# serviceberry3/weiner_slamit_v2

Hardware: AMD Instinct MI355X
Metric: frames/sec ORB extract+match @640x480x8lvl (higher is better)
Workload: dtype u8; 1 GPU; BASELINE configs[1]: 640x480 8-level ORB extract (1000 features, FAST 20/7) + brute-force 256-bit Hamming best/second match vs the stream's previous frame; 256 independent streams per GPU per step; distinct_frame_pairs_per_gpu=16, parallelism=streams sharded over 1 GPU(s), no data-path collective

## Files before the change

### weiner_slamit_v2_amd/csrc/orb_kernels.hip

```cpp
#include <hip/hip_runtime.h>
#include <stdint.h>

#include <algorithm>

#include "orb_types.h"
#include "slamit_math.h"
#include "wave_ops.h"
#include "../../include/slamit.h"
#include "../../include/slamit_orb_pattern.h"

#define WAVE 64

__global__ __launch_bounds__(256) void resize_level_kernel(
    const uint8_t* __restrict__ src, int sw, int sh, size_t sstride, size_t sframe,
    uint8_t* __restrict__ dst, int dw, int dh, size_t dstride, size_t dframe,
    const int* __restrict__ xofs, const short* __restrict__ ialpha,
    const int* __restrict__ yofs, const short* __restrict__ ibeta) {
    const int x4 = (blockIdx.x * 64 + (threadIdx.x & 63)) * 4;
    const int y = blockIdx.y * 4 + (threadIdx.x >> 6);
    const int f = blockIdx.z;
    if (x4 >= dw || y >= dh) return;
    const uint8_t* S = src + (size_t)f * sframe;
    int sy = yofs[y];
    int sy0 = min(max(sy, 0), sh - 1), sy1 = min(max(sy + 1, 0), sh - 1);
// ... 1119 lines not shown
    }
#endif
}

template <int OCT_NT>
__global__ __launch_bounds__(OCT_NT) void octree_kernel(
    const OrbLevel* __restrict__ levels, int nlevels,
    const unsigned long long* __restrict__ cand, size_t cand_frame_stride,
    int* __restrict__ cand_count,
    uint32_t* __restrict__ ws_xy, uint16_t* __restrict__ ws_node,
    OrbLevelKp* __restrict__ lkp, size_t kp_frame_stride, int* __restrict__ kp_count,
    int node_cap, int key_cap, int level_override ) {
    extern __shared__ __attribute__((aligned(16))) unsigned char smem[];
    __shared__ int wave_tmp[OCT_NT / 64];
    __shared__ int s_vars[4];
    uint32_t* k_xy = reinterpret_cast<uint32_t*>(smem + orbk_octree_node_bytes(node_cap));
    uint16_t* k_nd = reinterpret_cast<uint16_t*>(k_xy + key_cap);
    const int level = level_override >= 0 ? level_override : blockIdx.y;
    const int frame = blockIdx.x;
    const OrbLevel& L = levels[level];
    const int kidx = frame * nlevels + level;
    const int n_raw = cand_count[kidx * ORB_CC_PAD];
    const int n_keys = min(n_raw, L.cand_cap);
    __syncthreads();
    if (threadIdx.x == 0) { cand_count[kidx * ORB_CC_PAD] = 0; cand_count[kidx * ORB_CC_PAD + 1] = n_raw; }
    const unsigned long long* K = cand + L.cand_off + (size_t)frame * cand_frame_stride;
    OrbLevelKp* OUT = lkp + L.kp_off + (size_t)frame * kp_frame_stride;
    if (n_keys == 0) {
        if (threadIdx.x == 0) kp_count[kidx] = 0;
        return;
    }
    if (n_keys <= key_cap)
        octree_body<OCT_NT, true>(L, K, n_keys, k_xy, k_nd, OUT, &kp_count[kidx], smem, node_cap, wave_tmp, s_vars);
    else
        octree_body<OCT_NT, false>(L, K, n_keys, ws_xy + L.cand_off + (size_t)frame * cand_frame_stride,
                                        ws_node + L.cand_off + (size_t)frame * cand_frame_stride, OUT, &kp_count[kidx], smem,
                                        node_cap, wave_tmp, s_vars);
}

struct DiscTable { signed char uv[64][32]; int n; };
__constant__ DiscTable c_disc;

static DiscTable make_disc() {
    static const int umax[16] = {15, 15, 15, 15, 14, 14, 14, 13, 13, 12, 11, 10, 9, 8, 6, 3};
    DiscTable t;
    for (int l = 0; l < 64; ++l) for (int k = 0; k < 32; ++k) t.uv[l][k] = 0;
    t.n = 0;
    for (int v = -15; v <= 15; ++v)
        for (int u = -umax[v < 0 ? -v : v]; u <= umax[v < 0 ? -v : v]; ++u) {
            t.uv[t.n & 63][2 * (t.n >> 6)] = (signed char)u; t.uv[t.n & 63][2 * (t.n >> 6) + 1] = (signed char)v;
            ++t.n;
        }
    return t;
}

#define IC_KP_PER_WAVE 8
#define IC_R 15
#define IC_ROWS (2 * IC_R + 1)
#define IC_PITCH 32

__global__ __launch_bounds__(256) void ic_angle_kernel(
    const OrbLevel* __restrict__ levels, int nlevels,
    const uint8_t* __restrict__ img0, size_t img0_stride, size_t img0_frame,
    const uint8_t* __restrict__ pyr,
    OrbLevelKp* __restrict__ lkp, size_t kp_frame_stride, const int* __restrict__ kp_count, int xcd_frames, int kblocks) {
    const int lane = threadIdx.x & 63;
    int level, frame, kb;
    if (xcd_frames) {
        const unsigned w = blockIdx.x, k = w >> 3, P = (unsigned)(nlevels * kblocks), fq = k / P, local = k - fq * P;
        frame = (int)(8u * fq + ((w + fq) & 7u));
        if (frame >= xcd_frames) return;
        level = (int)(local / (unsigned)kblocks); kb = (int)(local - (unsigned)level * (unsigned)kblocks);
    } else { level = blockIdx.y; frame = blockIdx.z; kb = blockIdx.x; }
    const OrbLevel& L = levels[level];
    const int count = kp_count[frame * nlevels + level];
    const int i0 = (kb * 4 + (threadIdx.x >> 6)) * IC_KP_PER_WAVE;
    if (i0 >= count) return;
    const uint8_t* src;
    int stride;
    if (level == 0) { src = img0 + (size_t)frame * img0_frame; stride = (int)img0_stride; }
    else { src = pyr + L.plane_off + (size_t)frame * L.plane_bytes; stride = L.stride; }
    __shared__ __attribute__((aligned(16))) uint8_t s_win[4][IC_KP_PER_WAVE][IC_ROWS * IC_PITCH];
    const int wvi = threadIdx.x >> 6;
    OrbLevelKp* kp0 = lkp + L.kp_off + (size_t)frame * kp_frame_stride;
    typedef unsigned ic_u4 __attribute__((ext_vector_type(4), aligned(1)));
    {
        const int lr = min(lane >> 1, IC_ROWS - 1), lc = lane & 1;
        const unsigned loff = __umul24((unsigned)lr, (unsigned)stride) + 16u * (unsigned)lc;
        ic_u4 ld[IC_KP_PER_WAVE];
#pragma unroll
        for (int k = 0; k < IC_KP_PER_WAVE; ++k) {
            const int i = min(i0 + k, count - 1);
            const uint8_t* corner = src + (__umul24((unsigned)(kp0[i].y - IC_R), (unsigned)stride) + (unsigned)(kp0[i].x - IC_R));
            ld[k] = *reinterpret_cast<const ic_u4*>(corner + loff);
        }
#pragma unroll
        for (int k = 0; k < IC_KP_PER_WAVE; ++k)
            if (lane < 2 * IC_ROWS) *reinterpret_cast<uint4*>(&s_win[wvi][k][lr * IC_PITCH + 16 * lc]) = make_uint4(ld[k].x, ld[k].y, ld[k].z, ld[k].w);
    }
    int off[12], wu[12], wv[12];
    {
        const uint4 t0 = *reinterpret_cast<const uint4*>(&c_disc.uv[lane][0]);
        const uint2 t1 = *reinterpret_cast<const uint2*>(&c_disc.uv[lane][16]);
        const uint32_t tw[6] = {t0.x, t0.y, t0.z, t0.w, t1.x, t1.y};
#pragma unroll
        for (int j = 0; j < 12; ++j) {
            const uint32_t pr = tw[j >> 1] >> (16 * (j & 1));
            const int u = (int)(signed char)(pr & 0xFFu), v = (int)(signed char)((pr >> 8) & 0xFFu);
            off[j] = (v + IC_R) * IC_PITCH + (u + IC_R); wu[j] = u; wv[j] = v;
        }
    }
    const float factorPI = (float)(3.14159265358979323846 / 180.f);
    wave_sync_lds();
    int val[IC_KP_PER_WAVE][12];
#pragma unroll
    for (int k = 0; k < IC_KP_PER_WAVE; ++k)
#pragma unroll
        for (int j = 0; j < 12; ++j) val[k][j] = s_win[wvi][k][off[j]];
    int V[2 * IC_KP_PER_WAVE];
#pragma unroll
    for (int k = 0; k < IC_KP_PER_WAVE; ++k) {
        int m10 = 0, m01 = 0;
#pragma unroll
        for (int j = 0; j < 12; ++j) { m10 += __mul24(wu[j], val[k][j]); m01 += __mul24(wv[j], val[k][j]); }
        V[2 * k] = m10; V[2 * k + 1] = m01;
    }
    {
        const bool b0 = lane & 1, b1 = lane & 2, b2 = lane & 4, b3 = lane & 8;
#pragma unroll
        for (int p = 0; p < 8; ++p) { const int a = V[2 * p], b = V[2 * p + 1]; V[p] = (b0 ? b : a) + dpp<0xB1>(b0 ? a : b); }
#pragma unroll
        for (int p = 0; p < 4; ++p) { const int a = V[2 * p], b = V[2 * p + 1]; V[p] = (b1 ? b : a) + dpp<0x4E>(b1 ? a : b); }
#pragma unroll
        for (int p = 0; p < 2; ++p) { const int a = V[2 * p], b = V[2 * p + 1]; V[p] = (b2 ? b : a) + dpp<0x1B>(dpp<0x141>(b2 ? a : b)); }
        { const int a = V[0], b = V[1]; V[0] = (b3 ? b : a) + dpp<0x141>(dpp<0x140>(b3 ? a : b)); }
    }
    __shared__ int s_rows[4][64];
    int* sr = s_rows[threadIdx.x >> 6];
    sr[lane] = V[0];
    wave_sync_lds();
    const int tot = (sr[lane & 15] + sr[(lane & 15) + 16]) + (sr[(lane & 15) + 32] + sr[(lane & 15) + 48]);
    const int my10 = tot, my01 = dpp<0xB1>(tot);
    if (lane < 2 * IC_KP_PER_WAVE && !(lane & 1) && i0 + (lane >> 1) < count) {
        const float ang = slamit_fast_atan2((float)my01, (float)my10);
        float sn, cs;
        slamit_sincosf(ang * factorPI, &sn, &cs);
        OrbLevelKp* kp = kp0 + i0 + (lane >> 1);
        kp->angle = ang; kp->cs = cs; kp->sn = sn;
    }
}

__device__ __forceinline__ int reflect101(int p, int len) {
    p = p < 0 ? -p : p;
    p = p >= len ? 2 * len - 2 - p : p;
    return min(max(p, 0), len - 1);
}


typedef unsigned short blur_us2 __attribute__((ext_vector_type(2)));
__device__ __forceinline__ uint32_t udot2(uint32_t a, uint32_t b, uint32_t c) {
    return __builtin_amdgcn_udot2(__builtin_bit_cast(blur_us2, a), __builtin_bit_cast(blur_us2, b), c, false);
}

__device__ __forceinline__ uint32_t blur_fetch(const uint8_t* S, unsigned sstride, bool whole, int w, int h, int gx0, int row) {
    const unsigned ro = (unsigned)reflect101(row, h) * sstride;
    if (whole) return *reinterpret_cast<const uint32_t*>(S + (ro + (unsigned)gx0));
    if (gx0 >= w + 3) return 0u;
    uint32_t v = 0;
#pragma unroll
    for (int j = 0; j < 4; ++j) v |= (uint32_t)S[ro + (unsigned)reflect101(gx0 + j, w)] << (8 * j);
    return v;
}

struct BlurCol { unsigned a0, a1, sel; };
__device__ __forceinline__ BlurCol blur_col(int g, int w, unsigned ss) {
#define BLUR_SEL(i0, i1, i2, i3) ((unsigned)(i0) | ((unsigned)(i1) << 8) | ((unsigned)(i2) << 16) | ((unsigned)(i3) << 24))
    BlurCol c;
    if (g < 0) { c.a0 = 0u; c.a1 = 4u; c.sel = BLUR_SEL(4, 3, 2, 1); }
    else if (g + 4 <= w) { c.a0 = c.a1 = (unsigned)g; c.sel = BLUR_SEL(0, 1, 2, 3); }
    else if (g < w) {
        const int q = w - g;
        unsigned idx[4];
#pragma unroll
        for (int j = 0; j < 4; ++j) idx[j] = (unsigned)(j < q ? 4 + j : 2 * q + 2 - j);
        c.a0 = (unsigned)(g - 4); c.a1 = (unsigned)g; c.sel = BLUR_SEL(idx[0], idx[1], idx[2], idx[3]);
    } else if (g <= w + 2) {
        const int t = g - w, gb = (w - 4) & ~3;
        unsigned idx[4];
#pragma unroll
        for (int j = 0; j < 4; ++j) idx[j] = j <= 2 - t ? (unsigned)(w - 2 - t - j - gb) : 0x0Cu;
        c.a0 = (unsigned)gb; c.a1 = min((unsigned)gb + 4u, ss - 4u); c.sel = BLUR_SEL(idx[0], idx[1], idx[2], idx[3]);
    } else { c.a0 = c.a1 = 0u; c.sel = BLUR_SEL(0x0C, 0x0C, 0x0C, 0x0C); }
#undef BLUR_SEL
    return c;
}
__device__ __forceinline__ uint32_t blur_fetch2(const uint8_t* S, unsigned ss, int h, int row, const BlurCol c) {
    const unsigned ro = __umul24((unsigned)reflect101(row, h), ss);
    return __builtin_amdgcn_perm(*reinterpret_cast<const uint32_t*>(S + (ro + c.a1)), *reinterpret_cast<const uint32_t*>(S + (ro + c.a0)), c.sel);
}

template <bool INTERIOR>
__device__ __forceinline__ void blur_strip(uint8_t (*in)[72], uint32_t (*rp)[64], const uint8_t* S, const size_t sstride, const bool aligned,
                                           uint8_t* D, const unsigned dstride, const int w, const int h, const int bx, const int by0, const int tid) {
    const int i0 = tid, i1 = tid + 256;
    const bool has1 = i1 < 22 * 18;
    const int r0 = i0 / 18, r1 = i1 / 18;
    const int g0 = bx - 4 + 4 * (i0 - r0 * 18), g1 = bx - 4 + 4 * (i1 - r1 * 18);
    const bool whole0 = aligned && g0 >= 0 && g0 + 4 <= w, whole1 = aligned && g1 >= 0 && g1 + 4 <= w;
    uint32_t* const st0 = reinterpret_cast<uint32_t*>(&in[r0][4 * (i0 - r0 * 18)]);
    uint32_t* const st1 = reinterpret_cast<uint32_t*>(&in[has1 ? r1 : 0][has1 ? 4 * (i1 - r1 * 18) : 0]);
    const unsigned ss = (unsigned)sstride;
    const BlurCol bc0 = blur_col(g0, w, ss), bc1 = blur_col(g1, w, ss);
    uint32_t v0 = INTERIOR ? *reinterpret_cast<const uint32_t*>(S + (__umul24((unsigned)(by0 + r0 - 3), ss) + (unsigned)g0))
                           : aligned ? blur_fetch2(S, ss, h, by0 + r0 - 3, bc0) : blur_fetch(S, ss, whole0, w, h, g0, by0 + r0 - 3);
    uint32_t v1 = !has1 ? 0u : INTERIOR ? *reinterpret_cast<const uint32_t*>(S + (__umul24((unsigned)(by0 + r1 - 3), ss) + (unsigned)g1))
                                        : aligned ? blur_fetch2(S, ss, h, by0 + r1 - 3, bc1) : blur_fetch(S, ss, whole1, w, h, g1, by0 + r1 - 3);
    *st0 = v0;
    if (has1) *st1 = v1;
    __syncthreads();
    const uint32_t TA = 18u | (34u << 8) | (49u << 16) | (55u << 24), TB = 49u | (34u << 8) | (18u << 16);
    const int cy = tid >> 4, cx4 = (tid & 15) * 4;
    const bool odd = cy & 1;
    const uint32_t k0 = odd ? (18u << 16) : (18u | (34u << 16)), k1 = odd ? (34u | (49u << 16)) : (49u | (55u << 16));
    const uint32_t k2 = odd ? (55u | (49u << 16)) : (49u | (34u << 16)), k3 = odd ? (34u | (18u << 16)) : 18u;
#pragma unroll 1
    for (int s = 0; s < BLUR_STEPS; ++s) {
        const int by = by0 + 16 * s;
        const bool more = s + 1 < BLUR_STEPS && (INTERIOR || by + 16 < h);
        if (more) {
            if (INTERIOR) {
                v0 = *reinterpret_cast<const uint32_t*>(S + (__umul24((unsigned)(by + 16 + r0 - 3), ss) + (unsigned)g0));
                if (has1) v1 = *reinterpret_cast<const uint32_t*>(S + (__umul24((unsigned)(by + 16 + r1 - 3), ss) + (unsigned)g1));
            } else {
                if (aligned) {
                    v0 = blur_fetch2(S, ss, h, by + 16 + r0 - 3, bc0);
                    if (has1) v1 = blur_fetch2(S, ss, h, by + 16 + r1 - 3, bc1);
                } else {
                    v0 = blur_fetch(S, ss, whole0, w, h, g0, by + 16 + r0 - 3);
                    if (has1) v1 = blur_fetch(S, ss, whole1, w, h, g1, by + 16 + r1 - 3);
                }
            }
        }
        if (tid < 11 * 16) {
            const int p = tid >> 4, c = (tid & 15) * 4;
            uint32_t o[2][4];
#pragma unroll
            for (int rr = 0; rr < 2; ++rr) {
                const uint32_t* pw = reinterpret_cast<const uint32_t*>(&in[2 * p + rr][c]);
                const uint32_t w0 = pw[0], w1 = pw[1], w2 = pw[2];
                o[rr][0] = __builtin_amdgcn_udot4(__builtin_amdgcn_alignbyte(w2, w1, 1), TB, __builtin_amdgcn_udot4(__builtin_amdgcn_alignbyte(w1, w0, 1), TA, 0u, false), false);
                o[rr][1] = __builtin_amdgcn_udot4(__builtin_amdgcn_alignbyte(w2, w1, 2), TB, __builtin_amdgcn_udot4(__builtin_amdgcn_alignbyte(w1, w0, 2), TA, 0u, false), false);
                o[rr][2] = __builtin_amdgcn_udot4(__builtin_amdgcn_alignbyte(w2, w1, 3), TB, __builtin_amdgcn_udot4(__builtin_amdgcn_alignbyte(w1, w0, 3), TA, 0u, false), false);
                o[rr][3] = __builtin_amdgcn_udot4(w2, TB, __builtin_amdgcn_udot4(w1, TA, 0u, false), false);
            }
            *reinterpret_cast<uint4*>(&rp[p][c]) = make_uint4(o[0][0] | (o[1][0] << 16), o[0][1] | (o[1][1] << 16),
                                                               o[0][2] | (o[1][2] << 16), o[0][3] | (o[1][3] << 16));
        }
        __syncthreads();
        if (more) {
            *st0 = v0;
            if (has1) *st1 = v1;
        }
        if (INTERIOR || (bx + cx4 < w && by + cy < h)) {
            const int pb = cy >> 1;
            const uint4 a0 = *reinterpret_cast<const uint4*>(&rp[pb][cx4]), a1 = *reinterpret_cast<const uint4*>(&rp[pb + 1][cx4]);
            const uint4 a2 = *reinterpret_cast<const uint4*>(&rp[pb + 2][cx4]), a3 = *reinterpret_cast<const uint4*>(&rp[pb + 3][cx4]);
#define BLUR_COL(f) min((udot2(a3.f, k3, udot2(a2.f, k2, udot2(a1.f, k1, udot2(a0.f, k0, 1u << 15)))) >> 16), 255u)
            const uint32_t out = BLUR_COL(x) | (BLUR_COL(y) << 8) | (BLUR_COL(z) << 16) | (BLUR_COL(w) << 24);
#undef BLUR_COL
            *reinterpret_cast<uint32_t*>(D + (__umul24((unsigned)(by + cy), dstride) + (unsigned)(bx + cx4))) = out;
        }
        if (!more) break;
        __syncthreads();
    }
}

__global__ __launch_bounds__(256) void blur_all_kernel(
    const OrbLevel* __restrict__ levels, const uint4* __restrict__ tiles,
    const uint8_t* __restrict__ img0, size_t img0_stride, size_t img0_frame,
    const uint8_t* __restrict__ pyr, uint8_t* __restrict__ blur, unsigned ntiles, unsigned inv_tiles, unsigned total) {
    __shared__ __attribute__((aligned(16))) uint8_t in[22][72];
    __shared__ __attribute__((aligned(16))) uint32_t rp[11][64];
    const int tid = threadIdx.x;
    const unsigned lin = blockIdx.x, per_xcd = (total + 7u) >> 3;
    const unsigned logical = (lin & 7u) * per_xcd + (lin >> 3);
    if (logical >= total) return;
    int frame = (int)__umulhi(logical, inv_tiles);
    if ((unsigned)frame * ntiles > logical) --frame;
    const uint4 tt = tiles[logical - (unsigned)frame * ntiles];
    const int level = (int)tt.x, bx = (int)tt.y, by0 = (int)tt.z;
    const OrbLevel& L = levels[level];
    const int w = L.w, h = L.h;
    const uint8_t* S;
    size_t sstride;
    if (level == 0) { S = img0 + (size_t)frame * img0_frame; sstride = img0_stride; }
    else { S = pyr + L.plane_off + (size_t)frame * L.plane_bytes; sstride = (size_t)L.stride; }
    const bool aligned = ((((uintptr_t)S) | sstride) & 3) == 0;
    uint8_t* D = blur + L.blur_off + (size_t)frame * L.blur_bytes;
    const bool interior = aligned && bx >= 4 && bx + 68 <= w && by0 >= 3 && by0 + ORB_BLUR_STRIP_H + 3 <= h;
    if (interior) blur_strip<true>(in, rp, S, sstride, aligned, D, (unsigned)L.stride, w, h, bx, by0, tid);
    else blur_strip<false>(in, rp, S, sstride, aligned, D, (unsigned)L.stride, w, h, bx, by0, tid);
}

template <bool EDGE>
__global__ __launch_bounds__(256) void blur_stream_kernel(
    const OrbLevel* __restrict__ levels, const uint4* __restrict__ tiles,
    const uint8_t* __restrict__ img0, size_t img0_stride, size_t img0_frame,
    const uint8_t* __restrict__ pyr, uint8_t* __restrict__ blur, unsigned ntiles) {
    const unsigned tile = blockIdx.x * 16u + (threadIdx.x >> 4);
    if (tile >= ntiles) return;
    const int frame = blockIdx.y;
    const uint4 tt = tiles[tile];
    const int level = (int)tt.x, by0 = (int)tt.z;
    const int x0 = (int)tt.y + 4 * (int)(threadIdx.x & 15);
    const OrbLevel& L = levels[level];
    const int h = L.h;
    const uint8_t* S;
    unsigned ss;
    if (level == 0) { S = img0 + (size_t)frame * img0_frame; ss = (unsigned)img0_stride; }
    else { S = pyr + L.plane_off + (size_t)frame * L.plane_bytes; ss = (unsigned)L.stride; }
    if (EDGE && x0 >= L.w) return;
    BlurCol bc[3];
    if (EDGE) {
#pragma unroll
        for (int k = 0; k < 3; ++k) bc[k] = blur_col(x0 - 4 + 4 * k, L.w, ss);
    } else S += x0 - 4;
    uint8_t* D = blur + L.blur_off + (size_t)frame * L.blur_bytes + x0;
    const unsigned ds = (unsigned)L.stride;
    const uint32_t TA = 18u | (34u << 8) | (49u << 16) | (55u << 24), TB = 49u | (34u << 8) | (18u << 16);
    const uint32_t kA0 = 18u | (34u << 16), kA1 = 49u | (55u << 16), kA2 = 49u | (34u << 16), kA3 = 18u;
    const uint32_t kB0 = 18u << 16, kB1 = 34u | (49u << 16), kB2 = 55u | (49u << 16), kB3 = 34u | (18u << 16);
    const int ylast = min(by0 + ORB_BLUR_STRIP_H, h) - 1;
    const int p0 = (by0 - 3) >> 1, p1 = (ylast + 3) >> 1;
    typedef unsigned blur_u3 __attribute__((ext_vector_type(3)));
    auto fetch = [&](int yy) -> blur_u3 {
        int r = yy < 0 ? -yy : yy;
        r = r >= h ? 2 * h - 2 - r : r;
        r = min(max(r, 0), h - 1);
        if (EDGE) {
            const uint8_t* R = S + __umul24((unsigned)r, ss);
            blur_u3 v;
            v.x = __builtin_amdgcn_perm(*reinterpret_cast<const uint32_t*>(R + bc[0].a1), *reinterpret_cast<const uint32_t*>(R + bc[0].a0), bc[0].sel);
            v.y = __builtin_amdgcn_perm(*reinterpret_cast<const uint32_t*>(R + bc[1].a1), *reinterpret_cast<const uint32_t*>(R + bc[1].a0), bc[1].sel);
            v.z = __builtin_amdgcn_perm(*reinterpret_cast<const uint32_t*>(R + bc[2].a1), *reinterpret_cast<const uint32_t*>(R + bc[2].a0), bc[2].sel);
            return v;
        }
        return *reinterpret_cast<const blur_u3*>(S + __umul24((unsigned)r, ss));
    };
    auto rowpass = [&](const blur_u3 v, uint32_t* o) {
        o[0] = __builtin_amdgcn_udot4(__builtin_amdgcn_alignbyte(v.z, v.y, 1), TB, __builtin_amdgcn_udot4(__builtin_amdgcn_alignbyte(v.y, v.x, 1), TA, 0u, false), false);
        o[1] = __builtin_amdgcn_udot4(__builtin_amdgcn_alignbyte(v.z, v.y, 2), TB, __builtin_amdgcn_udot4(__builtin_amdgcn_alignbyte(v.y, v.x, 2), TA, 0u, false), false);
        o[2] = __builtin_amdgcn_udot4(__builtin_amdgcn_alignbyte(v.z, v.y, 3), TB, __builtin_amdgcn_udot4(__builtin_amdgcn_alignbyte(v.y, v.x, 3), TA, 0u, false), false);
        o[3] = __builtin_amdgcn_udot4(v.z, TB, __builtin_amdgcn_udot4(v.y, TA, 0u, false), false);
    };
    uint32_t P0[4] = {0, 0, 0, 0}, P1[4] = {0, 0, 0, 0}, P2[4] = {0, 0, 0, 0}, P3[4];
    blur_u3 va = fetch(2 * p0), vb = fetch(2 * p0 + 1), va1 = fetch(2 * p0 + 2), vb1 = fetch(2 * p0 + 3), va2 = fetch(2 * p0 + 4), vb2 = fetch(2 * p0 + 5);
#pragma unroll 4
    for (int p = p0; p <= p1; ++p) {
        const blur_u3 ca = va, cb = vb;
        va = va1; vb = vb1; va1 = va2; vb1 = vb2;
        va2 = fetch(2 * p + 6); vb2 = fetch(2 * p + 7);
        uint32_t oa[4], ob[4];
        rowpass(ca, oa); rowpass(cb, ob);
#pragma unroll
        for (int j = 0; j < 4; ++j) P3[j] = oa[j] | (ob[j] << 16);
        const int ya = 2 * p - 3, yb = 2 * p - 2;
#define BLUR_OUT(k0, k1, k2, k3, j) min((udot2(P3[j], k3, udot2(P2[j], k2, udot2(P1[j], k1, udot2(P0[j], k0, 1u << 15)))) >> 16), 255u)
        if (ya >= by0 && ya <= ylast)
            *reinterpret_cast<uint32_t*>(D + __umul24((unsigned)ya, ds)) = BLUR_OUT(kA0, kA1, kA2, kA3, 0) | (BLUR_OUT(kA0, kA1, kA2, kA3, 1) << 8) | (BLUR_OUT(kA0, kA1, kA2, kA3, 2) << 16) | (BLUR_OUT(kA0, kA1, kA2, kA3, 3) << 24);
        if (yb >= by0 && yb <= ylast)
            *reinterpret_cast<uint32_t*>(D + __umul24((unsigned)yb, ds)) = BLUR_OUT(kB0, kB1, kB2, kB3, 0) | (BLUR_OUT(kB0, kB1, kB2, kB3, 1) << 8) | (BLUR_OUT(kB0, kB1, kB2, kB3, 2) << 16) | (BLUR_OUT(kB0, kB1, kB2, kB3, 3) << 24);
#undef BLUR_OUT
#pragma unroll
        for (int j = 0; j < 4; ++j) { P0[j] = P1[j]; P1[j] = P2[j]; P2[j] = P3[j]; }
    }
}

__constant__ __attribute__((aligned(16))) signed char c_pattern[SLAMIT_ORB_PATTERN_INTS];
#define DESC_KP_PER_WAVE 4
#define DESC_R 18
#define DESC_ROWS (2 * DESC_R + 1)
#define DESC_PITCH 48
#define DESC_LOADS 2

__global__ __launch_bounds__(256) void describe_kernel(
    const OrbLevel* __restrict__ levels, int nlevels,
    const uint8_t* __restrict__ blur,
    const OrbLevelKp* __restrict__ lkp, size_t kp_frame_stride, const int* __restrict__ kp_count,
    slamit_kp* __restrict__ out_kps, uint8_t* __restrict__ out_desc, int out_cap,
    int* __restrict__ out_n, int xcd_frames , int kblocks) {
    const int lane = threadIdx.x & 63;
    int level, frame, kb;
    if (xcd_frames) {
        const unsigned w = blockIdx.x, k = w >> 3, P = (unsigned)(nlevels * kblocks), fq = k / P, local = k - fq * P;
        frame = (int)(8u * fq + ((w + fq) & 7u));
        if (frame >= xcd_frames) return;
        level = (int)(local / (unsigned)kblocks); kb = (int)(local - (unsigned)level * (unsigned)kblocks);
    } else { level = blockIdx.y; frame = blockIdx.z; kb = blockIdx.x; }
    const int i0 = (kb * 4 + (threadIdx.x >> 6)) * DESC_KP_PER_WAVE;
    const OrbLevel& L = levels[level];
    const int* counts = kp_count + frame * nlevels;
    int offset = 0, total = 0;
    for (int l = 0; l < nlevels; ++l) {
        int c = counts[l];
        if (l < level) offset += c;
        total += c;
    }
    if (level == 0 && i0 == 0 && lane == 0) out_n[frame] = min(total, out_cap);
    const int count = counts[level];
    if (i0 >= count) return;
    const int4 pw = reinterpret_cast<const int4*>(c_pattern)[lane];
    const int pt[4] = {pw.x, pw.y, pw.z, pw.w};
    float px0[4], py0[4], px1[4], py1[4];
#pragma unroll
    for (int t = 0; t < 4; ++t) {
        px0[t] = (float)(signed char)(pt[t] & 0xFF); py0[t] = (float)(signed char)((pt[t] >> 8) & 0xFF);
        px1[t] = (float)(signed char)((pt[t] >> 16) & 0xFF); py1[t] = (float)(signed char)((pt[t] >> 24) & 0xFF);
    }
    const uint8_t* img = blur + L.blur_off + (size_t)frame * L.blur_bytes;
    const unsigned step = (unsigned)L.stride;
    const OrbLevelKp* KP = lkp + L.kp_off + (size_t)frame * kp_frame_stride;
    OrbLevelKp kp[DESC_KP_PER_WAVE];
#pragma unroll
    for (int k = 0; k < DESC_KP_PER_WAVE; ++k) kp[k] = KP[min(i0 + k, count - 1)];
    __shared__ __attribute__((aligned(16))) uint8_t s_patch[4][DESC_KP_PER_WAVE][DESC_ROWS * DESC_PITCH];
    const int wv = threadIdx.x >> 6;
    int lrow[DESC_LOADS], lcol[DESC_LOADS];
    unsigned poff[DESC_LOADS];
#pragma unroll
    for (int it = 0; it < DESC_LOADS; ++it) {
        const int idx = lane + 64 * it;
        lrow[it] = (int)(((unsigned)idx * 21846u) >> 16);
        lcol[it] = idx - 3 * lrow[it];
        poff[it] = __umul24((unsigned)min(lrow[it], DESC_ROWS - 1), step) + 16u * (unsigned)lcol[it];
    }
    const __amdgpu_buffer_rsrc_t rsrc = __builtin_amdgcn_make_buffer_rsrc(const_cast<uint8_t*>(img), 0, (unsigned)L.stride * (unsigned)L.h, 0x00020000);
    typedef unsigned desc_u4 __attribute__((ext_vector_type(4)));
    desc_u4 ld[DESC_KP_PER_WAVE][DESC_LOADS];
#pragma unroll
    for (int k = 0; k < DESC_KP_PER_WAVE; ++k) {
        const unsigned base = __umul24((unsigned)(kp[k].y - DESC_R), step) + (unsigned)((kp[k].x - DESC_R) & ~3);
#pragma unroll
        for (int it = 0; it < DESC_LOADS; ++it) ld[k][it] = __builtin_amdgcn_raw_buffer_load_b128(rsrc, (int)(base + poff[it]), 0, 0);
    }
#pragma unroll
    for (int k = 0; k < DESC_KP_PER_WAVE; ++k)
#pragma unroll
        for (int it = 0; it < DESC_LOADS; ++it)
            if (lrow[it] < DESC_ROWS) *reinterpret_cast<desc_u4*>(&s_patch[wv][k][__mul24(lrow[it], DESC_PITCH) + 16 * lcol[it]]) = ld[k][it];
    __builtin_amdgcn_fence(__ATOMIC_ACQ_REL, "wavefront");
    __builtin_amdgcn_wave_barrier();
    typedef float desc_f2 __attribute__((ext_vector_type(2)));
    const desc_f2 magic = {12582912.0f, 12582912.0f};
    const unsigned DESC_BIAS = 0x400000u * (unsigned)DESC_PITCH + 0x4B400000u;
    int tv0[DESC_KP_PER_WAVE][4], tv1[DESC_KP_PER_WAVE][4];
#pragma unroll
    for (int k = 0; k < DESC_KP_PER_WAVE; ++k) {
        const float a = kp[k].cs, b = kp[k].sn;
        const desc_f2 ba = {b, a}, anb = {a, -b};
        const uint8_t* center = &s_patch[wv][k][DESC_R * DESC_PITCH + DESC_R + ((kp[k].x - DESC_R) & 3)];
        const uint8_t* biased = center - DESC_BIAS;
#pragma unroll
        for (int t = 0; t < 4; ++t) {
            const desc_f2 p0 = {px0[t], px0[t]}, q0 = {py0[t], py0[t]}, p1 = {px1[t], px1[t]}, q1 = {py1[t], py1[t]};
            const desc_f2 m0 = (p0 * ba + q0 * anb) + magic, m1 = (p1 * ba + q1 * anb) + magic;
            tv0[k][t] = biased[__umul24(__float_as_uint(m0.x), (unsigned)DESC_PITCH) + __float_as_uint(m0.y)];
            tv1[k][t] = biased[__umul24(__float_as_uint(m1.x), (unsigned)DESC_PITCH) + __float_as_uint(m1.y)];
        }
    }
#pragma unroll
    for (int k = 0; k < DESC_KP_PER_WAVE; ++k) {
        const int i = i0 + k, o = offset + i;
        unsigned nib = 0;
#pragma unroll
        for (int t = 0; t < 4; ++t) nib |= (unsigned)(tv0[k][t] < tv1[k][t]) << t;
        unsigned other = __shfl_xor(nib, 1, WAVE);
        if (i >= count || o >= out_cap) continue;
        if ((lane & 1) == 0)
            out_desc[((size_t)frame * out_cap + o) * SLAMIT_DESC_BYTES + (lane >> 1)] = (uint8_t)(nib | (other << 4));
        if (lane == 0) {
            slamit_kp kk;
            float fx = (float)kp[k].x, fy = (float)kp[k].y;
            if (level != 0) { fx *= L.scale; fy *= L.scale; }
            kk.x = fx; kk.y = fy; kk.size = L.patch_size; kk.angle = kp[k].angle; kk.response = kp[k].response;
            kk.octave = level; kk.class_id = -1;
            out_kps[(size_t)frame * out_cap + o] = kk;
        }
    }
}

__global__ __launch_bounds__(256) void pad_level_kernel(const uint8_t* __restrict__ src, int w, int h,
                                                        size_t sstride, uint8_t* __restrict__ dst) {
    const int B = SLAMIT_EDGE_THRESHOLD;
    const int pw = w + 2 * B, ph = h + 2 * B;
    int x = blockIdx.x * 64 + (threadIdx.x & 63), y = blockIdx.y * 4 + (threadIdx.x >> 6);
    if (x >= pw || y >= ph) return;
    dst[(size_t)y * pw + x] = src[(size_t)reflect101(y - B, h) * sstride + reflect101(x - B, w)];
}

__global__ void decode_candidates_kernel(const OrbLevel* __restrict__ levels, int level,
                                         const unsigned long long* __restrict__ K, int n,
                                         unsigned long long* __restrict__ order_out, int* __restrict__ xys) {
    int k = blockIdx.x * blockDim.x + threadIdx.x;
    if (k >= n) return;
    const OrbLevel& L = levels[level];
    unsigned long long c = K[k];
    unsigned order = (unsigned)c;
    int lx = order & 63, ly = (order >> 6) & 63, cell = order >> 12;
    int ci = cell / L.nCols, cj = cell - ci * L.nCols;
    xys[3 * k + 0] = cj * L.wCell + lx;
    xys[3 * k + 1] = ci * L.hCell + ly;
    xys[3 * k + 2] = (int)(c >> 32);
    order_out[k] = order;
}

extern "C++" {

hipError_t orbk_upload_pattern(hipStream_t st) {
    static const DiscTable disc = make_disc();
    hipError_t e = hipMemcpyToSymbolAsync(HIP_SYMBOL(c_disc), &disc, sizeof(disc), 0, hipMemcpyHostToDevice, st);
    if (e != hipSuccess) return e;
    return hipMemcpyToSymbolAsync(HIP_SYMBOL(c_pattern), slamit_orb_pattern, SLAMIT_ORB_PATTERN_INTS, 0,
                                  hipMemcpyHostToDevice, st);
}

void orbk_resize(hipStream_t st, const uint8_t* src, int sw, int sh, size_t sstride, size_t sframe,
                 uint8_t* dst, int dw, int dh, size_t dstride, size_t dframe, const int* xofs,
                 const short* ialpha, const int* yofs, const short* ibeta, int nframes) {
    dim3 grid((dw + 255) / 256, (dh + 3) / 4, nframes);
    hipLaunchKernelGGL(resize_level_kernel, grid, dim3(256), 0, st, src, sw, sh, sstride, sframe, dst, dw,
                       dh, dstride, dframe, xofs, ialpha, yofs, ibeta);
}

hipError_t orbk_pyramid_prepare(int smem_bytes) {
    return hipFuncSetAttribute(reinterpret_cast<const void*>(pyramid_fused_kernel),
                               hipFuncAttributeMaxDynamicSharedMemorySize, smem_bytes);
}

void orbk_pyramid(hipStream_t st, const OrbLevel* levels, int nlevels, const PyrBox* boxes, const PyrTabs* tabs,
                  int nregions, const uint8_t* img0, size_t img0_stride, size_t img0_frame, uint8_t* pyr, int bufA_bytes,
                  int smem_bytes, int nframes, int l_first, int l_last) {
    hipLaunchKernelGGL(pyramid_fused_kernel, dim3(nregions, nframes), dim3(PYR_THREADS), smem_bytes, st, levels, nlevels, boxes,
                       tabs, img0, img0_stride, img0_frame, pyr, bufA_bytes, l_first, l_last);
}

#ifndef FAST_PS
#define FAST_PS 48
#define FAST_PL 80
#endif
static int fast_pitch(int max_wcell) { return max_wcell + 11 <= FAST_PS ? FAST_PS : FAST_PL; }

size_t orbk_fast_smem(int max_wcell, int max_hcell) {
    const int P = fast_pitch(max_wcell);
    const int tile_rows = max_hcell + 6, sc_rows = max_hcell + 2;
    const int kp_cap = ((max_wcell + 1) / 2) * ((max_hcell + 1) / 2);
    return (size_t)4 * fast_wave_bytes(P, tile_rows, sc_rows, kp_cap);
}

hipError_t orbk_fast_prepare(int max_wcell, int max_hcell) {
    const int smem = (int)orbk_fast_smem(max_wcell, max_hcell);
    hipError_t e;
    if (fast_pitch(max_wcell) == FAST_PS) {
        e = hipFuncSetAttribute(reinterpret_cast<const void*>(fast_cells_kernel<FAST_PS>), hipFuncAttributeMaxDynamicSharedMemorySize, smem);
    } else {
        e = hipFuncSetAttribute(reinterpret_cast<const void*>(fast_cells_kernel<FAST_PL>), hipFuncAttributeMaxDynamicSharedMemorySize, smem);
    }
    return e;
}

void orbk_fast(hipStream_t st, const FastTab& tab, int nlevels, const uint32_t* d_cells, int cells_per_frame,
               const uint8_t* img0, size_t img0_stride, size_t img0_frame, const uint8_t* pyr,
               unsigned long long* cand, size_t cand_frame_stride, int* cand_count, int iniTh, int minTh,
               int max_wcell, int max_hcell, int nframes) {
    const int tile_rows = max_hcell + 6, sc_rows = max_hcell + 2;
    const int kp_cap = ((max_wcell + 1) / 2) * ((max_hcell + 1) / 2);
    const int wpb = cells_per_frame < 1600 ? 1 : 4;
    const int xcd_frames = nframes >= 16 ? nframes : 0;
    const dim3 grid = xcd_frames ? dim3((unsigned)(((nframes + 7) / 8) * 8) * (unsigned)((cells_per_frame + wpb - 1) / wpb))
                                 : dim3(wpb == 1 ? (unsigned)((cells_per_frame + 31) & ~31) : (unsigned)((cells_per_frame + wpb - 1) / wpb), nframes);
    const size_t smem = orbk_fast_smem(max_wcell, max_hcell) / 4 * wpb;
    if (fast_pitch(max_wcell) == FAST_PS)
        hipLaunchKernelGGL(fast_cells_kernel<FAST_PS>, grid, dim3(64 * wpb), smem, st, tab, reinterpret_cast<const uint4*>(d_cells), nlevels, cells_per_frame, img0,
                           (unsigned)img0_stride, img0_frame, pyr, cand, cand_frame_stride, cand_count, iniTh, minTh, tile_rows,
                           sc_rows, kp_cap, xcd_frames);
    else
        hipLaunchKernelGGL(fast_cells_kernel<FAST_PL>, grid, dim3(64 * wpb), smem, st, tab, reinterpret_cast<const uint4*>(d_cells), nlevels, cells_per_frame, img0,
                           (unsigned)img0_stride, img0_frame, pyr, cand, cand_frame_stride, cand_count, iniTh, minTh, tile_rows,
                           sc_rows, kp_cap, xcd_frames);
}

hipError_t orbk_octree_prepare(int node_cap, int key_cap) {
    static int prepared = 0;
    const int want = (int)orbk_octree_smem(node_cap, key_cap);
    if (want <= prepared) return hipSuccess;
    prepared = want;
    hipError_t e = hipFuncSetAttribute(reinterpret_cast<const void*>(octree_kernel<256>), hipFuncAttributeMaxDynamicSharedMemorySize, want);
    if (e != hipSuccess) return e;
    e = hipFuncSetAttribute(reinterpret_cast<const void*>(octree_kernel<OCT_THREADS>), hipFuncAttributeMaxDynamicSharedMemorySize, want);
    if (e != hipSuccess) return e;
    return hipFuncSetAttribute(reinterpret_cast<const void*>(octree_kernel<1024>), hipFuncAttributeMaxDynamicSharedMemorySize, want);
}

void orbk_octree(hipStream_t st, const OrbLevel* levels, int nlevels, const unsigned long long* cand,
                 size_t cand_frame_stride, int* cand_count, uint32_t* ws_xy, uint16_t* ws_node,
                 OrbLevelKp* lkp, size_t kp_frame_stride, int* kp_count, int node_cap, int key_cap, int nframes,
                 int level_override) {
    dim3 grid(nframes, level_override >= 0 ? 1 : nlevels);
    const int nt = nframes >= 96 ? 256 : nframes <= 16 ? 1024 : OCT_THREADS;
    if (nframes >= 96) key_cap = std::min(key_cap, 2048);
    if (nt == 1024)
        hipLaunchKernelGGL(octree_kernel<1024>, grid, dim3(1024), orbk_octree_smem(node_cap, key_cap), st, levels, nlevels, cand,
                           cand_frame_stride, cand_count, ws_xy, ws_node, lkp, kp_frame_stride, kp_count, node_cap,
                           key_cap, level_override);
    else if (nt == 256)
        hipLaunchKernelGGL(octree_kernel<256>, grid, dim3(256), orbk_octree_smem(node_cap, key_cap), st, levels, nlevels, cand,
                           cand_frame_stride, cand_count, ws_xy, ws_node, lkp, kp_frame_stride, kp_count, node_cap,
                           key_cap, level_override);
    else
        hipLaunchKernelGGL(octree_kernel<OCT_THREADS>, grid, dim3(OCT_THREADS), orbk_octree_smem(node_cap, key_cap), st, levels, nlevels, cand,
                           cand_frame_stride, cand_count, ws_xy, ws_node, lkp, kp_frame_stride, kp_count, node_cap,
                           key_cap, level_override);
}

void orbk_ic_angle(hipStream_t st, const OrbLevel* levels, int nlevels, const uint8_t* img0,
                   size_t img0_stride, size_t img0_frame, const uint8_t* pyr, OrbLevelKp* lkp,
                   size_t kp_frame_stride, const int* kp_count, int max_kp, int nframes) {
    const int kblocks = (max_kp + 4 * IC_KP_PER_WAVE - 1) / (4 * IC_KP_PER_WAVE);
    if (nframes >= 16)
        hipLaunchKernelGGL(ic_angle_kernel, dim3((unsigned)(((nframes + 7) / 8) * 8 * nlevels * kblocks)), dim3(256), 0, st, levels,
                           nlevels, img0, img0_stride, img0_frame, pyr, lkp, kp_frame_stride, kp_count, nframes, kblocks);
    else
        hipLaunchKernelGGL(ic_angle_kernel, dim3(kblocks, nlevels, nframes), dim3(256), 0, st, levels,
                           nlevels, img0, img0_stride, img0_frame, pyr, lkp, kp_frame_stride, kp_count, 0, kblocks);
}

void orbk_blur_stream(hipStream_t st, const OrbLevel* levels, const uint32_t* d_tiles, int ntiles, const uint8_t* img0,
                      size_t img0_stride, size_t img0_frame, const uint8_t* pyr, uint8_t* blur, int nframes, bool edge) {
    if (ntiles <= 0) return;
    if (edge)
        hipLaunchKernelGGL(blur_stream_kernel<true>, dim3((ntiles + 15) / 16, nframes), dim3(256), 0, st, levels, reinterpret_cast<const uint4*>(d_tiles), img0,
                           img0_stride, img0_frame, pyr, blur, (unsigned)ntiles);
    else
        hipLaunchKernelGGL(blur_stream_kernel<false>, dim3((ntiles + 15) / 16, nframes), dim3(256), 0, st, levels, reinterpret_cast<const uint4*>(d_tiles), img0,
                           img0_stride, img0_frame, pyr, blur, (unsigned)ntiles);
}

void orbk_blur(hipStream_t st, const OrbLevel* levels, const uint32_t* d_tiles, int total_tiles, const uint8_t* img0,
               size_t img0_stride, size_t img0_frame, const uint8_t* pyr, uint8_t* blur, int nframes) {
    if (total_tiles <= 0) return;
    const unsigned total = (unsigned)total_tiles * (unsigned)nframes, grid = ((total + 7u) >> 3) << 3;
    const unsigned inv = (unsigned)((0x100000000ull + (unsigned)total_tiles - 1) / (unsigned)total_tiles);
    hipLaunchKernelGGL(blur_all_kernel, dim3(grid), dim3(256), 0, st, levels, reinterpret_cast<const uint4*>(d_tiles), img0,
                       img0_stride, img0_frame, pyr, blur, (unsigned)total_tiles, inv, total);
}

void orbk_describe(hipStream_t st, const OrbLevel* levels, int nlevels, const uint8_t* blur,
                   const OrbLevelKp* lkp, size_t kp_frame_stride, const int* kp_count, slamit_kp* out_kps,
                   uint8_t* out_desc, int out_cap, int* out_n, int max_kp, int nframes) {
    const int kblocks = (max_kp + 4 * DESC_KP_PER_WAVE - 1) / (4 * DESC_KP_PER_WAVE);
    if (nframes >= 16)
        hipLaunchKernelGGL(describe_kernel, dim3((unsigned)(((nframes + 7) / 8) * 8 * nlevels * kblocks)), dim3(256), 0, st, levels,
                           nlevels, blur, lkp, kp_frame_stride, kp_count, out_kps, out_desc, out_cap, out_n, nframes, kblocks);
    else
        hipLaunchKernelGGL(describe_kernel, dim3(kblocks, nlevels, nframes), dim3(256), 0, st, levels,
                           nlevels, blur, lkp, kp_frame_stride, kp_count, out_kps, out_desc, out_cap, out_n, 0, kblocks);
}

void orbk_pad(hipStream_t st, const uint8_t* src, int w, int h, size_t sstride, uint8_t* dst) {
    hipLaunchKernelGGL(pad_level_kernel, dim3((w + 38 + 63) / 64, (h + 38 + 3) / 4), dim3(256), 0, st, src, w, h,
                       sstride, dst);
}

void orbk_decode_candidates(hipStream_t st, const OrbLevel* levels, int level, const unsigned long long* K,
                            int n, unsigned long long* order_out, int* xys) {
    if (n <= 0) return;
    hipLaunchKernelGGL(decode_candidates_kernel, dim3((n + 255) / 256), dim3(256), 0, st, levels, level, K, n,
                       order_out, xys);
}

}
```

Baseline: 316,700 frames/s.

## Widen blur stream lanes to eight pixels with direct dot-product row taps

Generalizes the streaming Gaussian blur kernel so each lane produces 8 output pixels instead of 4, with 8 lanes per 64-pixel strip and 32 strips per workgroup. This amortizes the halo words each lane fetches and the row-index arithmetic over more pixels. The horizontal pass now multiplies the raw input words by precomputed shifted-tap constants instead of byte-aligning the data first, and output packing uses packed 16-bit min plus perm. The cost is a wider register window and more live registers per lane, which may lower occupancy.

```diff
diff --git a/weiner_slamit_v2_amd/csrc/orb_kernels.hip b/weiner_slamit_v2_amd/csrc/orb_kernels.hip
--- a/weiner_slamit_v2_amd/csrc/orb_kernels.hip
+++ b/weiner_slamit_v2_amd/csrc/orb_kernels.hip
@@ -1445,17 +1445,37 @@
     else blur_strip<false>(in, rp, S, sstride, aligned, D, (unsigned)L.stride, w, h, bx, by0, tid);
 }
 
+#ifndef BLUR_LANE_PX
+#define BLUR_LANE_PX 8
+#endif
+#ifndef BLUR_PAIRS_AHEAD
+#define BLUR_PAIRS_AHEAD 3
+#endif
+#define BLUR_NW (BLUR_LANE_PX / 4 + 2)
+#define BLUR_LANES (64 / BLUR_LANE_PX)
+#define BLUR_WG_STRIPS (256 / BLUR_LANES)
+static_assert(BLUR_LANE_PX == 4 || BLUR_LANE_PX == 8, "BLUR_LANE_PX");
+static_assert(BLUR_PAIRS_AHEAD == 2 || BLUR_PAIRS_AHEAD == 3, "BLUR_PAIRS_AHEAD");
+struct BlurWin { uint32_t d[BLUR_NW]; };
+constexpr uint32_t blur_ktap(int m) {
+    constexpr uint32_t T[7] = {18, 34, 49, 55, 49, 34, 18};
+    uint32_t k = 0;
+    for (int b = 0; b < 4; ++b)
+        if (b - m >= 0 && b - m <= 6) k |= T[b - m] << (8 * b);
+    return k;
+}
+typedef unsigned short blur_pk16 __attribute__((ext_vector_type(2)));
 template <bool EDGE>
 __global__ __launch_bounds__(256) void blur_stream_kernel(
     const OrbLevel* __restrict__ levels, const uint4* __restrict__ tiles,
     const uint8_t* __restrict__ img0, size_t img0_stride, size_t img0_frame,
     const uint8_t* __restrict__ pyr, uint8_t* __restrict__ blur, unsigned ntiles) {
-    const unsigned tile = blockIdx.x * 16u + (threadIdx.x >> 4);
+    const unsigned tile = blockIdx.x * (unsigned)BLUR_WG_STRIPS + (threadIdx.x / BLUR_LANES);
     if (tile >= ntiles) return;
     const int frame = blockIdx.y;
     const uint4 tt = tiles[tile];
     const int level = (int)tt.x, by0 = (int)tt.z;
-    const int x0 = (int)tt.y + 4 * (int)(threadIdx.x & 15);
+    const int x0 = (int)tt.y + BLUR_LANE_PX * (int)(threadIdx.x % BLUR_LANES);
     const OrbLevel& L = levels[level];
     const int h = L.h;
     const uint8_t* S;
@@ -1463,59 +1483,92 @@
     if (level == 0) { S = img0 + (size_t)frame * img0_frame; ss = (unsigned)img0_stride; }
     else { S = pyr + L.plane_off + (size_t)frame * L.plane_bytes; ss = (unsigned)L.stride; }
     if (EDGE && x0 >= L.w) return;
-    BlurCol bc[3];
+    BlurCol bc[BLUR_NW];
     if (EDGE) {
 #pragma unroll
-        for (int k = 0; k < 3; ++k) bc[k] = blur_col(x0 - 4 + 4 * k, L.w, ss);
+        for (int k = 0; k < BLUR_NW; ++k) bc[k] = blur_col(x0 - 4 + 4 * k, L.w, ss);
     } else S += x0 - 4;
     uint8_t* D = blur + L.blur_off + (size_t)frame * L.blur_bytes + x0;
     const unsigned ds = (unsigned)L.stride;
-    const uint32_t TA = 18u | (34u << 8) | (49u << 16) | (55u << 24), TB = 49u | (34u << 8) | (18u << 16);
     const uint32_t kA0 = 18u | (34u << 16), kA1 = 49u | (55u << 16), kA2 = 49u | (34u << 16), kA3 = 18u;
     const uint32_t kB0 = 18u << 16, kB1 = 34u | (49u << 16), kB2 = 55u | (49u << 16), kB3 = 34u | (18u << 16);
     const int ylast = min(by0 + ORB_BLUR_STRIP_H, h) - 1;
     const int p0 = (by0 - 3) >> 1, p1 = (ylast + 3) >> 1;
-    typedef unsigned blur_u3 __attribute__((ext_vector_type(3)));
-    auto fetch = [&](int yy) -> blur_u3 {
+    auto fetch = [&](int yy) -> BlurWin {
         int r = yy < 0 ? -yy : yy;
         r = r >= h ? 2 * h - 2 - r : r;
         r = min(max(r, 0), h - 1);
+        const uint8_t* R = S + __umul24((unsigned)r, ss);
+        BlurWin v;
         if (EDGE) {
-            const uint8_t* R = S + __umul24((unsigned)r, ss);
-            blur_u3 v;
-            v.x = __builtin_amdgcn_perm(*reinterpret_cast<const uint32_t*>(R + bc[0].a1), *reinterpret_cast<const uint32_t*>(R + bc[0].a0), bc[0].sel);
-            v.y = __builtin_amdgcn_perm(*reinterpret_cast<const uint32_t*>(R + bc[1].a1), *reinterpret_cast<const uint32_t*>(R + bc[1].a0), bc[1].sel);
-            v.z = __builtin_amdgcn_perm(*reinterpret_cast<const uint32_t*>(R + bc[2].a1), *reinterpret_cast<const uint32_t*>(R + bc[2].a0), bc[2].sel);
-            return v;
-        }
-        return *reinterpret_cast<const blur_u3*>(S + __umul24((unsigned)r, ss));
+#pragma unroll
+            for (int k = 0; k < BLUR_NW; ++k)
+                v.d[k] = __builtin_amdgcn_perm(*reinterpret_cast<const uint32_t*>(R + bc[k].a1), *reinterpret_cast<const uint32_t*>(R + bc[k].a0), bc[k].sel);
+        } else __builtin_memcpy(&v, __builtin_assume_aligned(R, 4), sizeof v);
+        return v;
     };
-    auto rowpass = [&](const blur_u3 v, uint32_t* o) {
-        o[0] = __builtin_amdgcn_udot4(__builtin_amdgcn_alignbyte(v.z, v.y, 1), TB, __builtin_amdgcn_udot4(__builtin_amdgcn_alignbyte(v.y, v.x, 1), TA, 0u, false), false);
-        o[1] = __builtin_amdgcn_udot4(__builtin_amdgcn_alignbyte(v.z, v.y, 2), TB, __builtin_amdgcn_udot4(__builtin_amdgcn_alignbyte(v.y, v.x, 2), TA, 0u, false), false);
-        o[2] = __builtin_amdgcn_udot4(__builtin_amdgcn_alignbyte(v.z, v.y, 3), TB, __builtin_amdgcn_udot4(__builtin_amdgcn_alignbyte(v.y, v.x, 3), TA, 0u, false), false);
-        o[3] = __builtin_amdgcn_udot4(v.z, TB, __builtin_amdgcn_udot4(v.y, TA, 0u, false), false);
+    auto rowpass = [&](const BlurWin& v, uint32_t* o) {
+#pragma unroll
+        for (int j = 0; j < BLUR_LANE_PX; ++j) {
+#ifdef BLUR_SHIFT_DATA
+            const uint32_t TA = 18u | (34u << 8) | (49u << 16) | (55u << 24), TB = 49u | (34u << 8) | (18u << 16);
+            const int q = j >> 2, r = (j & 3) + 1;
+            const uint32_t lo = r == 4 ? v.d[q + 1] : __builtin_amdgcn_alignbyte(v.d[q + 1], v.d[q], r);
+            const uint32_t hi = r == 4 ? v.d[q + 2] : __builtin_amdgcn_alignbyte(v.d[q + 2], v.d[q + 1], r);
+            o[j] = __builtin_amdgcn_udot4(hi, TB, __builtin_amdgcn_udot4(lo, TA, 0u, false), false);
+#else
+            uint32_t acc = 0u;
+#pragma unroll
+            for (int d = 0; d < BLUR_NW; ++d)
+                if (blur_ktap(j + 1 - 4 * d) != 0u) acc = __builtin_amdgcn_udot4(v.d[d], blur_ktap(j + 1 - 4 * d), acc, false);
+            o[j] = acc;
+#endif
+        }
     };
-    uint32_t P0[4] = {0, 0, 0, 0}, P1[4] = {0, 0, 0, 0}, P2[4] = {0, 0, 0, 0}, P3[4];
-    blur_u3 va = fetch(2 * p0), vb = fetch(2 * p0 + 1), va1 = fetch(2 * p0 + 2), vb1 = fetch(2 * p0 + 3), va2 = fetch(2 * p0 + 4), vb2 = fetch(2 * p0 + 5);
+    uint32_t P0[BLUR_LANE_PX] = {}, P1[BLUR_LANE_PX] = {}, P2[BLUR_LANE_PX] = {}, P3[BLUR_LANE_PX];
+    auto pack4 = [&](const uint32_t* a) -> uint32_t {
+#ifdef BLUR_DOT_CLAMP
+        return __builtin_amdgcn_perm(a[1], a[0], 0x0C0C0602u) | __builtin_amdgcn_perm(a[3], a[2], 0x06020C0Cu);
+#endif
+        const uint32_t lim = 0x00FF00FFu;
+        const uint32_t h01 = __builtin_amdgcn_perm(a[1], a[0], 0x07060302u), h23 = __builtin_amdgcn_perm(a[3], a[2], 0x07060302u);
+        const uint32_t m01 = __builtin_bit_cast(uint32_t, __builtin_elementwise_min(__builtin_bit_cast(blur_pk16, h01), __builtin_bit_cast(blur_pk16, lim)));
+        const uint32_t m23 = __builtin_bit_cast(uint32_t, __builtin_elementwise_min(__builtin_bit_cast(blur_pk16, h23), __builtin_bit_cast(blur_pk16, lim)));
+        return __builtin_amdgcn_perm(m23, m01, 0x06040200u);
+    };
+    auto outrow = [&](int y, uint32_t k0, uint32_t k1, uint32_t k2, uint32_t k3) {
+        uint32_t a[BLUR_LANE_PX], o[BLUR_LANE_PX / 4];
+#pragma unroll
+#ifdef BLUR_DOT_CLAMP
+#define BLUR_DOT2(a, b, c) __builtin_amdgcn_udot2(__builtin_bit_cast(blur_us2, a), __builtin_bit_cast(blur_us2, b), c, true)
+        for (int j = 0; j < BLUR_LANE_PX; ++j) a[j] = BLUR_DOT2(P3[j], k3, BLUR_DOT2(P2[j], k2, BLUR_DOT2(P1[j], k1, BLUR_DOT2(P0[j], k0, 0xFF008000u))));
+#undef BLUR_DOT2
+#else
+        for (int j = 0; j < BLUR_LANE_PX; ++j) a[j] = udot2(P3[j], k3, udot2(P2[j], k2, udot2(P1[j], k1, udot2(P0[j], k0, 1u << 15))));
+#endif
+#pragma unroll
+        for (int q = 0; q < BLUR_LANE_PX / 4; ++q) o[q] = pack4(a + 4 * q);
+        __builtin_memcpy(__builtin_assume_aligned(D + __umul24((unsigned)y, ds), 4), o, sizeof o);
+    };
+    BlurWin va[BLUR_PAIRS_AHEAD], vb[BLUR_PAIRS_AHEAD];
+#pragma unroll
+    for (int i = 0; i < BLUR_PAIRS_AHEAD; ++i) { va[i] = fetch(2 * (p0 + i)); vb[i] = fetch(2 * (p0 + i) + 1); }
 #pragma unroll 4
     for (int p = p0; p <= p1; ++p) {
-        const blur_u3 ca = va, cb = vb;
-        va = va1; vb = vb1; va1 = va2; vb1 = vb2;
-        va2 = fetch(2 * p + 6); vb2 = fetch(2 * p + 7);
-        uint32_t oa[4], ob[4];
+        const BlurWin ca = va[0], cb = vb[0];
+#pragma unroll
+        for (int i = 0; i + 1 < BLUR_PAIRS_AHEAD; ++i) { va[i] = va[i + 1]; vb[i] = vb[i + 1]; }
+        va[BLUR_PAIRS_AHEAD - 1] = fetch(2 * (p + BLUR_PAIRS_AHEAD));
+        vb[BLUR_PAIRS_AHEAD - 1] = fetch(2 * (p + BLUR_PAIRS_AHEAD) + 1);
+        uint32_t oa[BLUR_LANE_PX], ob[BLUR_LANE_PX];
         rowpass(ca, oa); rowpass(cb, ob);
 #pragma unroll
-        for (int j = 0; j < 4; ++j) P3[j] = oa[j] | (ob[j] << 16);
+        for (int j = 0; j < BLUR_LANE_PX; ++j) P3[j] = oa[j] | (ob[j] << 16);
         const int ya = 2 * p - 3, yb = 2 * p - 2;
-#define BLUR_OUT(k0, k1, k2, k3, j) min((udot2(P3[j], k3, udot2(P2[j], k2, udot2(P1[j], k1, udot2(P0[j], k0, 1u << 15)))) >> 16), 255u)
-        if (ya >= by0 && ya <= ylast)
-            *reinterpret_cast<uint32_t*>(D + __umul24((unsigned)ya, ds)) = BLUR_OUT(kA0, kA1, kA2, kA3, 0) | (BLUR_OUT(kA0, kA1, kA2, kA3, 1) << 8) | (BLUR_OUT(kA0, kA1, kA2, kA3, 2) << 16) | (BLUR_OUT(kA0, kA1, kA2, kA3, 3) << 24);
-        if (yb >= by0 && yb <= ylast)
-            *reinterpret_cast<uint32_t*>(D + __umul24((unsigned)yb, ds)) = BLUR_OUT(kB0, kB1, kB2, kB3, 0) | (BLUR_OUT(kB0, kB1, kB2, kB3, 1) << 8) | (BLUR_OUT(kB0, kB1, kB2, kB3, 2) << 16) | (BLUR_OUT(kB0, kB1, kB2, kB3, 3) << 24);
-#undef BLUR_OUT
-#pragma unroll
-        for (int j = 0; j < 4; ++j) { P0[j] = P1[j]; P1[j] = P2[j]; P2[j] = P3[j]; }
+        if (ya >= by0 && ya <= ylast) outrow(ya, kA0, kA1, kA2, kA3);
+        if (yb >= by0 && yb <= ylast) outrow(yb, kB0, kB1, kB2, kB3);
+#pragma unroll
+        for (int j = 0; j < BLUR_LANE_PX; ++j) { P0[j] = P1[j]; P1[j] = P2[j]; P2[j] = P3[j]; }
     }
 }
 
@@ -1781,10 +1834,10 @@
                       size_t img0_stride, size_t img0_frame, const uint8_t* pyr, uint8_t* blur, int nframes, bool edge) {
     if (ntiles <= 0) return;
     if (edge)
-        hipLaunchKernelGGL(blur_stream_kernel<true>, dim3((ntiles + 15) / 16, nframes), dim3(256), 0, st, levels, reinterpret_cast<const uint4*>(d_tiles), img0,
+        hipLaunchKernelGGL(blur_stream_kernel<true>, dim3((ntiles + BLUR_WG_STRIPS - 1) / BLUR_WG_STRIPS, nframes), dim3(256), 0, st, levels, reinterpret_cast<const uint4*>(d_tiles), img0,
                            img0_stride, img0_frame, pyr, blur, (unsigned)ntiles);
     else
-        hipLaunchKernelGGL(blur_stream_kernel<false>, dim3((ntiles + 15) / 16, nframes), dim3(256), 0, st, levels, reinterpret_cast<const uint4*>(d_tiles), img0,
+        hipLaunchKernelGGL(blur_stream_kernel<false>, dim3((ntiles + BLUR_WG_STRIPS - 1) / BLUR_WG_STRIPS, nframes), dim3(256), 0, st, levels, reinterpret_cast<const uint4*>(d_tiles), img0,
                            img0_stride, img0_frame, pyr, blur, (unsigned)ntiles);
 }
 
```

New measurement: 299,600 frames/s. 5.4% lower.
